# MiniMax-AI/VTP

Measured on NVIDIA H100. Metric: images/sec (256x256 encode+decode+3-loss step), higher is better.
Workload: dtype bf16

## Files before the change

vtp_b200/csrc/attention_bwd.cu:

```cuda
#include <stdlib.h>

#include "attention_bwd.cuh"
#include "host.h"
#include "ptx.cuh"

namespace vtp {

static constexpr int AB_THREADS = 384;
static constexpr int BQ = 0, BK_ = 32768, BV = 65536, BDO = 98304, BP = 131072, BDS = 163840, BX = 196608;
static constexpr int X_P0 = 0, X_DS0 = 1056, X_DK0 = 2112, X_DV0 = 2368, X_PCOL = 2624, X_DSCOL = 3648, X_BAR = 4672;
static constexpr int AB_SMEM = BX + X_BAR + 128 + 1024;

struct AttnBwdDev {
    const __nv_bfloat16* qkv;
    const __nv_bfloat16* o;
    const __nv_bfloat16* dout;
    const float* lse;
    __nv_bfloat16* dqkv;
    const __nv_bfloat16* rope_sin;
    const __nv_bfloat16* rope_cos;
    int B, T, H, D, prefix, HW, causal, nkt;
    float scale, scale_log2;
    int pack, rprefix;
};
// ... 271 lines not shown
                    if (kj < HW) {
                        float f[64];
                        load_row64(smem + BK_, kj, f);
                        float s = 0.f;
#pragma unroll
                        for (int d = 0; d < 64; ++d) s += q0[d] * f[d];
                        load_row64(smem + BV, kj, f);
                        float dp = 0.f;
#pragma unroll
                        for (int d = 0; d < 64; ++d) dp += do0[d] * f[d];
                        pv = ex2f(s * p.scale_log2 - lse0);
                        dsv = p.scale * pv * (dp - delta0);
                    }
                    p0[kj] = pv, ds0[kj] = dsv;
                }
            }
            __syncwarp();
            if (lane == 0) mbar_arrive(bar_cls);
            float kc[64], vc[64];
            load_grow64(p.qkv + row0 * 3 * D + D + h * 64, kc);
            load_grow64(p.qkv + row0 * 3 * D + 2 * D + h * 64, vc);
            float s00 = 0.f, dp00 = 0.f;
#pragma unroll
            for (int d = 0; d < 64; ++d) s00 += q0[d] * kc[d], dp00 += do0[d] * vc[d];
            const float p00 = ex2f(s00 * p.scale_log2 - lse0);
            const float ds00 = p.scale * p00 * (dp00 - delta0);
            float a0 = 0.f, a1 = 0.f;
            for (int kj = 0; kj < HW; ++kj) {
                const float dsv = ds0[kj];
                const uint32_t w = *reinterpret_cast<const uint32_t*>(smem + BK_ + sw_off(kj, 2 * lane));
                a0 += dsv * bf16_lo(w), a1 += dsv * bf16_hi(w);
            }
            {
                const uint32_t w = __ldg(reinterpret_cast<const uint32_t*>(p.qkv + row0 * 3 * D + D + h * 64) + lane);
                a0 += ds00 * bf16_lo(w), a1 += ds00 * bf16_hi(w);
            }
            *reinterpret_cast<uint32_t*>(p.dqkv + row0 * 3 * D + h * 64 + 2 * lane) = pack_bf16x2(a0, a1);
            if (lane == 0) p0[260] = p00, ds0[260] = ds00;
        }
    }

    __syncthreads();
    if (warp == 8 && prefix > 0) {
        const float p00 = p0[260], ds00 = ds0[260];
        const uint32_t wdo = __ldg(reinterpret_cast<const uint32_t*>(p.dout + row0 * D + h * 64) + lane);
        const uint32_t wq = __ldg(reinterpret_cast<const uint32_t*>(p.qkv + row0 * 3 * D + h * 64) + lane);
        const float v0 = dv0[2 * lane] + p00 * bf16_lo(wdo), v1 = dv0[2 * lane + 1] + p00 * bf16_hi(wdo);
        const float k0 = dk0[2 * lane] + ds00 * bf16_lo(wq), k1 = dk0[2 * lane + 1] + ds00 * bf16_hi(wq);
        *reinterpret_cast<uint32_t*>(p.dqkv + row0 * 3 * D + 2 * D + h * 64 + 2 * lane) = pack_bf16x2(v0, v1);
        *reinterpret_cast<uint32_t*>(p.dqkv + row0 * 3 * D + D + h * 64 + 2 * lane) = pack_bf16x2(k0, k1);
    }
}


}

using namespace vtp;

extern "C" int vtp_attention_bwd(const void* qkv, const void* o, const void* dout, const float* lse, void* dqkv,
                                 const void* rope_sin, const void* rope_cos, int B, int T, int H, int prefix, int causal,
                                 vtp_stream_t st) {
    VTP_CHECK_ARG(qkv && o && dout && lse && dqkv && B > 0 && T > 0 && H > 0, "attention_bwd: bad args");
    VTP_CHECK_ARG(prefix == 0 || prefix == 1, "attention_bwd: prefix must be 0 or 1");
    VTP_CHECK_ARG(!(prefix && causal), "attention_bwd: causal + prefix is not supported");
    VTP_CHECK_ARG((rope_sin == nullptr) == (rope_cos == nullptr), "attention_bwd: rope tables");
    const int HW = T - prefix;
    VTP_CHECK_ARG(HW >= 1 && HW <= 256, "attention_bwd: %d non-prefix tokens not in [1,256]", HW);
    VTP_CHECK_ARG(B <= 65535, "attention_bwd: grid too large");
    const int D = H * 64;
    AttnBwdDev p;
    p.qkv = (const __nv_bfloat16*)qkv, p.o = (const __nv_bfloat16*)o, p.dout = (const __nv_bfloat16*)dout;
    p.lse = lse, p.dqkv = (__nv_bfloat16*)dqkv;
    p.rope_sin = (const __nv_bfloat16*)rope_sin, p.rope_cos = (const __nv_bfloat16*)rope_cos;
    p.B = B, p.T = T, p.H = H, p.D = D, p.prefix = prefix, p.HW = HW, p.causal = causal;
    p.nkt = HW > 128 ? 2 : 1;
    p.scale = 0.125f, p.scale_log2 = 0.125f * 1.4426950408889634f;
    p.pack = 0, p.rprefix = prefix;
    if (!causal && T <= 64 && B > 1 && getenv("VTP_ATTN_NO_PACK") == nullptr) {
        p.pack = 128 / T;
        p.prefix = 0, p.HW = T, p.nkt = 1;
    }
    CUtensorMap tq, td;
    {
        uint64_t dims[2] = {(uint64_t)3 * D, (uint64_t)B * T}, strides[1] = {(uint64_t)3 * D * 2};
        uint32_t box[2] = {64, 128};
        int rc = make_tmap_bf16(&tq, qkv, 2, dims, strides, box);
        if (rc) return rc;
    }
    {
        uint64_t dims[2] = {(uint64_t)D, (uint64_t)B * T}, strides[1] = {(uint64_t)D * 2};
        uint32_t box[2] = {64, 128};
        int rc = make_tmap_bf16(&td, dout, 2, dims, strides, box);
        if (rc) return rc;
    }
    static bool configured = false;
    if (!configured) {
        VTP_CUDA(cudaFuncSetAttribute(attn_bwd_kernel<1>, cudaFuncAttributeMaxDynamicSharedMemorySize, AB_SMEM));
        VTP_CUDA(cudaFuncSetAttribute(attn_bwd_kernel<2>, cudaFuncAttributeMaxDynamicSharedMemorySize, AB_SMEM));
        configured = true;
    }
    const dim3 grid(H, p.pack ? ceil_div(B, p.pack) : B);
    if (p.nkt == 2) attn_bwd_kernel<2><<<grid, AB_THREADS, AB_SMEM, (cudaStream_t)st>>>(tq, td, p);
    else attn_bwd_kernel<1><<<grid, AB_THREADS, AB_SMEM, (cudaStream_t)st>>>(tq, td, p);
    VTP_LAUNCH_CHECK();
    return VTP_OK;
}
```

vtp_b200/csrc/attention_bwd.cuh:

```cuda
#pragma once
#include "ptx.cuh"

namespace vtp {

__device__ __forceinline__ float ex2f(float x) {
    float y;
    asm("ex2.approx.ftz.f32 %0, %1;" : "=f"(y) : "f"(x));
    return y;
}
__device__ __forceinline__ uint32_t sw_off(int row, int col) {
    return row * 128 + ((((col >> 3) ^ (row & 7)) << 4) | ((col & 7) << 1));
}
__device__ __forceinline__ void load_row64(const uint8_t* tile, int row, float (&f)[64]) {
#pragma unroll
    for (int c = 0; c < 8; ++c) {
        const uint4 w = *reinterpret_cast<const uint4*>(tile + sw_off(row, c * 8));
        f[c * 8 + 0] = bf16_lo(w.x), f[c * 8 + 1] = bf16_hi(w.x), f[c * 8 + 2] = bf16_lo(w.y), f[c * 8 + 3] = bf16_hi(w.y);
        f[c * 8 + 4] = bf16_lo(w.z), f[c * 8 + 5] = bf16_hi(w.z), f[c * 8 + 6] = bf16_lo(w.w), f[c * 8 + 7] = bf16_hi(w.w);
    }
}
__device__ __forceinline__ void load_grow64(const __nv_bfloat16* g, float (&f)[64]) {
    const uint4* p = reinterpret_cast<const uint4*>(g);
#pragma unroll
    for (int c = 0; c < 8; ++c) {
        const uint4 w = __ldg(p + c);
        f[c * 8 + 0] = bf16_lo(w.x), f[c * 8 + 1] = bf16_hi(w.x), f[c * 8 + 2] = bf16_lo(w.y), f[c * 8 + 3] = bf16_hi(w.y);
        f[c * 8 + 4] = bf16_lo(w.z), f[c * 8 + 5] = bf16_hi(w.z), f[c * 8 + 6] = bf16_lo(w.w), f[c * 8 + 7] = bf16_hi(w.w);
    }
}

__device__ __forceinline__ float quad_dot(const uint8_t* tile, int row, const __nv_bfloat16* g, int c4) {
    float acc = 0.f;
#pragma unroll
    for (int c = 0; c < 2; ++c) {
        const uint4 a = *reinterpret_cast<const uint4*>(tile + sw_off(row, 16 * c4 + 8 * c));
        const uint4 w = __ldg(reinterpret_cast<const uint4*>(g + 16 * c4 + 8 * c));
        const uint32_t aw[4] = {a.x, a.y, a.z, a.w}, ww[4] = {w.x, w.y, w.z, w.w};
#pragma unroll
        for (int e = 0; e < 4; ++e) acc += bf16_lo(aw[e]) * bf16_lo(ww[e]) + bf16_hi(aw[e]) * bf16_hi(ww[e]);
    }
    acc += __shfl_xor_sync(0xffffffffu, acc, 1);
    acc += __shfl_xor_sync(0xffffffffu, acc, 2);
    return acc;
}

__device__ __forceinline__ void rope_bwd_frag(float (&g)[16], const __nv_bfloat16* sin_row, const __nv_bfloat16* cos_row, int c4) {
#pragma unroll
    for (int jn = 0; jn < 4; ++jn) {
        const int d = 8 * jn + 2 * c4;
        const uint32_t s_lo = __ldg(reinterpret_cast<const uint32_t*>(sin_row + d));
        const uint32_t s_hi = __ldg(reinterpret_cast<const uint32_t*>(sin_row + d + 32));
        const uint32_t c_lo = __ldg(reinterpret_cast<const uint32_t*>(cos_row + d));
        const uint32_t c_hi = __ldg(reinterpret_cast<const uint32_t*>(cos_row + d + 32));
        const float sl[2] = {bf16_lo(s_lo), bf16_hi(s_lo)}, sh[2] = {bf16_lo(s_hi), bf16_hi(s_hi)};
        const float cl[2] = {bf16_lo(c_lo), bf16_hi(c_lo)}, ch[2] = {bf16_lo(c_hi), bf16_hi(c_hi)};
#pragma unroll
        for (int c = 0; c < 2; ++c) {
            const float a = g[2 * jn + c], b = g[2 * (jn + 4) + c];
            g[2 * jn + c] = a * cl[c] + b * sh[c];
            g[2 * (jn + 4) + c] = b * ch[c] - a * sl[c];
        }
    }
}

}
```

vtp_b200/csrc/attention_bwd_long.cu:

```cuda
#include "attention_bwd.cuh"
#include "host.h"
#include "ptx.cuh"

namespace vtp {

namespace {

constexpr int BL_THREADS = 384;
constexpr int BL_NSTAGE = 2;
constexpr int BL_TILE = 128 * 128;
constexpr int DQ_Q = 0, DQ_DO = BL_TILE, DQ_KV = 2 * BL_TILE, DQ_BAR = DQ_KV + BL_NSTAGE * 2 * BL_TILE;
constexpr int DQ_SMEM = DQ_BAR + 128 + 1024;
constexpr int KV_K = 0, KV_V = BL_TILE, KV_QD = 2 * BL_TILE, KV_LD = KV_QD + BL_NSTAGE * 2 * BL_TILE;
constexpr int KV_BAR = KV_LD + BL_NSTAGE * 1024;
constexpr int KV_SMEM = KV_BAR + 128 + 1024;
constexpr float LOG2E = 1.4426950408889634f;

struct AttnBwdLongDev {
    const __nv_bfloat16* qkv;
    const __nv_bfloat16* o;
    const __nv_bfloat16* dout;
    const float* lse;
    float* delta;
    __nv_bfloat16* dqkv;
    const __nv_bfloat16* rope_sin;
    const __nv_bfloat16* rope_cos;
    int B, T, H, D, prefix, HW;
    float scale, scale_log2;
};

__global__ void __launch_bounds__(256) attn_bwd_delta_kernel(const AttnBwdLongDev p) {
    const long gid = (long)blockIdx.x * blockDim.x + threadIdx.x;
    const long pair = gid >> 3;
    const int c = (int)(gid & 7);
    const bool valid = pair < (long)p.B * p.T * p.H;
    float acc = 0.f;
    if (valid) {
        const long tok = pair / p.H;
        const int h = (int)(pair - tok * p.H);
        const uint4 a = __ldg(reinterpret_cast<const uint4*>(p.dout + tok * p.D + h * 64) + c);
        const uint4 w = __ldg(reinterpret_cast<const uint4*>(p.o + tok * p.D + h * 64) + c);
        const uint32_t aw[4] = {a.x, a.y, a.z, a.w}, ww[4] = {w.x, w.y, w.z, w.w};
#pragma unroll
        for (int e = 0; e < 4; ++e) acc += bf16_lo(aw[e]) * bf16_lo(ww[e]) + bf16_hi(aw[e]) * bf16_hi(ww[e]);
    }
    acc += __shfl_xor_sync(0xffffffffu, acc, 1);
    acc += __shfl_xor_sync(0xffffffffu, acc, 2);
    acc += __shfl_xor_sync(0xffffffffu, acc, 4);
    if (valid && c == 0) {
        const long tok = pair / p.H;
        const int h = (int)(pair - tok * p.H);
        const long b = tok / p.T;
        p.delta[(b * p.H + h) * p.T + (tok - b * p.T)] = acc;
    }
}

__device__ __forceinline__ void pack_a(const float (&x)[32], uint32_t (&a)[4][4]) {
#pragma unroll
    for (int kk = 0; kk < 4; ++kk) {
        a[kk][0] = pack_bf16x2(x[8 * kk], x[8 * kk + 1]), a[kk][1] = pack_bf16x2(x[8 * kk + 2], x[8 * kk + 3]);
        a[kk][2] = pack_bf16x2(x[8 * kk + 4], x[8 * kk + 5]), a[kk][3] = pack_bf16x2(x[8 * kk + 6], x[8 * kk + 7]);
    }
}

__global__ void __launch_bounds__(BL_THREADS, 1) attn_bwd_long_dq_kernel(const __grid_constant__ CUtensorMap tm_qkv,
                                                                          const __grid_constant__ CUtensorMap tm_do,
                                                                          const AttnBwdLongDev p) {
    extern __shared__ uint8_t smem_raw[];
    uint8_t* smem = reinterpret_cast<uint8_t*>((reinterpret_cast<uintptr_t>(smem_raw) + 1023) & ~uintptr_t(1023));
    uint64_t* bars = reinterpret_cast<uint64_t*>(smem + DQ_BAR);
    uint64_t* bar_q = bars;
    uint64_t* full = bars + 1;
    uint64_t* empty = full + BL_NSTAGE;

    const int warp = threadIdx.x >> 5, lane = threadIdx.x & 31;
    const int qt = blockIdx.x, h = blockIdx.y, b = blockIdx.z;
    const int D = p.D, T = p.T, prefix = p.prefix, HW = p.HW;
    const long row0 = (long)b * T;
    const int nkt = (HW + 127) / 128;

    if (threadIdx.x == 0) {
        tma_prefetch_desc(&tm_qkv);
        tma_prefetch_desc(&tm_do);
        mbar_init(bar_q, 1);
        for (int s = 0; s < BL_NSTAGE; ++s) mbar_init(full + s, 1), mbar_init(empty + s, 8);
        fence_barrier_init();
    }
    __syncthreads();

    if (warp < 8) {
        setmaxnreg_inc<200>();
        const int wg = warp >> 2, tw = threadIdx.x & 127, c4 = lane & 3;
        int rr[2], qi[2];
        bool qvalid[2];
#pragma unroll
        for (int i = 0; i < 2; ++i) {
            rr[i] = 64 * wg + 16 * (tw >> 5) + (lane >> 2) + 8 * i;
            qi[i] = 128 * qt + rr[i];
            qvalid[i] = qi[i] < HW;
        }
        const __nv_bfloat16* kcls = p.qkv + row0 * 3 * D + D + h * 64;
        const __nv_bfloat16* vcls = p.qkv + row0 * 3 * D + 2 * D + h * 64;
        mbar_wait(bar_q, 0);
        float lsc[2], dl[2], ds_cls[2];
#pragma unroll
        for (int i = 0; i < 2; ++i) {
            const long li = ((long)b * p.H + h) * T + prefix + qi[i];
            lsc[i] = qvalid[i] ? p.lse[li] * LOG2E : 0.f;
            dl[i] = qvalid[i] ? p.delta[li] : 0.f;
            ds_cls[i] = 0.f;
            if (prefix > 0) {
                const float s0 = quad_dot(smem + DQ_Q, rr[i], kcls, c4);
                const float dp0 = quad_dot(smem + DQ_DO, rr[i], vcls, c4);
                if (qvalid[i]) ds_cls[i] = p.scale * ex2f(s0 * p.scale_log2 - lsc[i]) * (dp0 - dl[i]);
            }
        }
        float dq[32];
// ... 1 lines not shown
        for (int k = 0; k < 32; ++k) dq[k] = 0.f;
        const uint32_t aQ = smem_u32(smem + DQ_Q) + wg * 8192, aDO = smem_u32(smem + DQ_DO) + wg * 8192;
        for (int t = 0; t < nkt; ++t) {
            const int st = t % BL_NSTAGE;
            mbar_wait(full + st, (t / BL_NSTAGE) & 1);
            const uint32_t aK = smem_u32(smem + DQ_KV + st * 2 * BL_TILE), aV = aK + BL_TILE;
            const int klim = HW - 128 * t;
#pragma unroll 1
            for (int half = 0; half < 2 && 64 * half < klim; ++half) {
                float s[32], dp[32];
                wgmma_fence();
#pragma unroll
                for (int j = 0; j < 4; ++j)
                    wgmma_m64n64_ss<0, 0>(s, wgmma_desc_sw128(aQ + j * 32, 0, 1024),
                                          wgmma_desc_sw128(aK + half * 8192 + j * 32, 0, 1024), j > 0);
#pragma unroll
                for (int j = 0; j < 4; ++j)
                    wgmma_m64n64_ss<0, 0>(dp, wgmma_desc_sw128(aDO + j * 32, 0, 1024),
                                          wgmma_desc_sw128(aV + half * 8192 + j * 32, 0, 1024), j > 0);
                wgmma_commit();
                wgmma_wait<0>();
                fence_regs(s);
                fence_regs(dp);
#pragma unroll
                for (int jn = 0; jn < 8; ++jn)
#pragma unroll
                    for (int i = 0; i < 2; ++i)
#pragma unroll
                        for (int c = 0; c < 2; ++c) {
                            const int e = 4 * jn + 2 * i + c;
                            float de = 0.f;
                            if (qvalid[i] && 64 * half + 8 * jn + 2 * c4 + c < klim) {
                                const float pe = ex2f(s[e] * p.scale_log2 - lsc[i]);
                                de = p.scale * pe * (dp[e] - dl[i]);
                            }
                            s[e] = de;
                        }
                uint32_t a[4][4];
                pack_a(s, a);
                wgmma_fence();
#pragma unroll
                for (int kk = 0; kk < 4; ++kk)
                    wgmma_m64n64_rs<1>(dq, a[kk], wgmma_desc_sw128(aK + (4 * half + kk) * 2048, 8192, 1024), 1);
                wgmma_commit();
                wgmma_wait<0>();
                fence_regs(dq);
            }
            __syncwarp();
            if (lane == 0) mbar_arrive(empty + st);
        }
#pragma unroll
        for (int i = 0; i < 2; ++i) {
            if (!qvalid[i]) continue;
            float gq[16];
#pragma unroll
            for (int e = 0; e < 16; ++e) gq[e] = dq[4 * (e >> 1) + 2 * i + (e & 1)];
            if (prefix > 0) {
#pragma unroll
                for (int jn = 0; jn < 8; ++jn) {
                    const uint32_t w = __ldg(reinterpret_cast<const uint32_t*>(kcls + 8 * jn + 2 * c4));
                    gq[2 * jn] += ds_cls[i] * bf16_lo(w), gq[2 * jn + 1] += ds_cls[i] * bf16_hi(w);
                }
            }
            if (p.rope_sin) rope_bwd_frag(gq, p.rope_sin + (long)qi[i] * 64, p.rope_cos + (long)qi[i] * 64, c4);
            __nv_bfloat16* drow = p.dqkv + (row0 + prefix + qi[i]) * 3 * D + h * 64;
#pragma unroll
            for (int jn = 0; jn < 8; ++jn)
                *reinterpret_cast<uint32_t*>(drow + 8 * jn + 2 * c4) = pack_bf16x2(gq[2 * jn], gq[2 * jn + 1]);
        }
    } else {
        setmaxnreg_dec<104>();
        if (warp != 8 || lane != 0) return;
        const int row_k = (int)row0 + prefix;
        mbar_expect_tx(bar_q, 2 * BL_TILE);
        tma_load_2d(smem + DQ_Q, &tm_qkv, bar_q, h * 64, row_k + 128 * qt);
        tma_load_2d(smem + DQ_DO, &tm_do, bar_q, h * 64, row_k + 128 * qt);
        for (int t = 0; t < nkt; ++t) {
            const int st = t % BL_NSTAGE;
            if (t >= BL_NSTAGE) mbar_wait(empty + st, ((t / BL_NSTAGE) - 1) & 1);
            uint8_t* kv = smem + DQ_KV + st * 2 * BL_TILE;
            mbar_expect_tx(full + st, 2 * BL_TILE);
            tma_load_2d(kv, &tm_qkv, full + st, D + h * 64, row_k + 128 * t);
            tma_load_2d(kv + BL_TILE, &tm_qkv, full + st, 2 * D + h * 64, row_k + 128 * t);
        }
    }
}

__global__ void __launch_bounds__(BL_THREADS, 1) attn_bwd_long_dkdv_kernel(const __grid_constant__ CUtensorMap tm_qkv,
                                                                            const __grid_constant__ CUtensorMap tm_do,
                                                                            const AttnBwdLongDev p) {
    extern __shared__ uint8_t smem_raw[];
    uint8_t* smem = reinterpret_cast<uint8_t*>((reinterpret_cast<uintptr_t>(smem_raw) + 1023) & ~uintptr_t(1023));
    uint64_t* bars = reinterpret_cast<uint64_t*>(smem + KV_BAR);
    uint64_t* bar_kv = bars;
    uint64_t* full = bars + 1;
    uint64_t* empty = full + BL_NSTAGE;

    const int warp = threadIdx.x >> 5, lane = threadIdx.x & 31;
    const int kt = blockIdx.x, h = blockIdx.y, b = blockIdx.z;
    const int D = p.D, T = p.T, prefix = p.prefix, HW = p.HW;
    const long row0 = (long)b * T;
    const int nqt = (HW + 127) / 128;
    const long lrow = ((long)b * p.H + h) * T;

    if (threadIdx.x == 0) {
        tma_prefetch_desc(&tm_qkv);
        tma_prefetch_desc(&tm_do);
        mbar_init(bar_kv, 1);
        for (int s = 0; s < BL_NSTAGE; ++s) mbar_init(full + s, 1 + 32), mbar_init(empty + s, 8);
        fence_barrier_init();
    }
    __syncthreads();

    if (warp < 8) {
        setmaxnreg_inc<200>();
        const int wg = warp >> 2, tw = threadIdx.x & 127, c4 = lane & 3;
        int rr[2], kj[2];
        bool kvalid[2];
#pragma unroll
        for (int i = 0; i < 2; ++i) {
            rr[i] = 64 * wg + 16 * (tw >> 5) + (lane >> 2) + 8 * i;
// ... 30 lines not shown
#pragma unroll 1
            for (int half = 0; half < 2 && 64 * half < qlim; ++half) {
                float s[32], dp[32];
                wgmma_fence();
#pragma unroll
                for (int j = 0; j < 4; ++j)
                    wgmma_m64n64_ss<0, 0>(s, wgmma_desc_sw128(aK + j * 32, 0, 1024),
                                          wgmma_desc_sw128(aQ + half * 8192 + j * 32, 0, 1024), j > 0);
#pragma unroll
                for (int j = 0; j < 4; ++j)
                    wgmma_m64n64_ss<0, 0>(dp, wgmma_desc_sw128(aV + j * 32, 0, 1024),
                                          wgmma_desc_sw128(aDO + half * 8192 + j * 32, 0, 1024), j > 0);
                wgmma_commit();
                wgmma_wait<0>();
                fence_regs(s);
                fence_regs(dp);
#pragma unroll
                for (int jn = 0; jn < 8; ++jn)
#pragma unroll
                    for (int c = 0; c < 2; ++c) {
                        const int qc = 64 * half + 8 * jn + 2 * c4 + c;
                        const float lq = lse_s[qc], dq = dl_s[qc];
#pragma unroll
                        for (int i = 0; i < 2; ++i) {
                            const int e = 4 * jn + 2 * i + c;
                            float pe = 0.f, de = 0.f;
                            if (kvalid[i] && qc < qlim) {
                                pe = ex2f(s[e] * p.scale_log2 - lq);
                                de = p.scale * pe * (dp[e] - dq);
                            }
                            s[e] = pe, dp[e] = de;
                        }
                    }
                uint32_t ap[4][4], as[4][4];
                pack_a(s, ap);
                pack_a(dp, as);
                wgmma_fence();
#pragma unroll
                for (int kk = 0; kk < 4; ++kk) {
                    wgmma_m64n64_rs<1>(dv, ap[kk], wgmma_desc_sw128(aDO + (4 * half + kk) * 2048, 8192, 1024), 1);
                    wgmma_m64n64_rs<1>(dk, as[kk], wgmma_desc_sw128(aQ + (4 * half + kk) * 2048, 8192, 1024), 1);
                }
                wgmma_commit();
                wgmma_wait<0>();
                fence_regs(dv);
                fence_regs(dk);
            }
            __syncwarp();
            if (lane == 0) mbar_arrive(empty + st);
        }
#pragma unroll
        for (int i = 0; i < 2; ++i) {
            if (!kvalid[i]) continue;
            float gv[16], gk[16];
#pragma unroll
            for (int e = 0; e < 16; ++e) {
                const int jn = e >> 1, cc = e & 1;
                gv[e] = dv[4 * jn + 2 * i + cc], gk[e] = dk[4 * jn + 2 * i + cc];
            }
            if (prefix > 0) {
#pragma unroll
                for (int jn = 0; jn < 8; ++jn) {
                    const uint32_t wd = __ldg(reinterpret_cast<const uint32_t*>(docls + 8 * jn + 2 * c4));
                    const uint32_t wq = __ldg(reinterpret_cast<const uint32_t*>(qcls + 8 * jn + 2 * c4));
                    gv[2 * jn] += p0j[i] * bf16_lo(wd), gv[2 * jn + 1] += p0j[i] * bf16_hi(wd);
                    gk[2 * jn] += ds0j[i] * bf16_lo(wq), gk[2 * jn + 1] += ds0j[i] * bf16_hi(wq);
                }
            }
            if (p.rope_sin) rope_bwd_frag(gk, p.rope_sin + (long)kj[i] * 64, p.rope_cos + (long)kj[i] * 64, c4);
            __nv_bfloat16* drow = p.dqkv + (row0 + prefix + kj[i]) * 3 * D + h * 64;
#pragma unroll
            for (int jn = 0; jn < 8; ++jn) {
                *reinterpret_cast<uint32_t*>(drow + 2 * D + 8 * jn + 2 * c4) = pack_bf16x2(gv[2 * jn], gv[2 * jn + 1]);
                *reinterpret_cast<uint32_t*>(drow + D + 8 * jn + 2 * c4) = pack_bf16x2(gk[2 * jn], gk[2 * jn + 1]);
            }
        }
    } else {
        setmaxnreg_dec<104>();
        if (warp != 8) return;
        const int row_k = (int)row0 + prefix;
        if (lane == 0) {
            mbar_expect_tx(bar_kv, 2 * BL_TILE);
            tma_load_2d(smem + KV_K, &tm_qkv, bar_kv, D + h * 64, row_k + 128 * kt);
            tma_load_2d(smem + KV_V, &tm_qkv, bar_kv, 2 * D + h * 64, row_k + 128 * kt);
        }
        for (int t = 0; t < nqt; ++t) {
            const int st = t % BL_NSTAGE;
            if (t >= BL_NSTAGE) mbar_wait(empty + st, ((t / BL_NSTAGE) - 1) & 1);
            if (lane == 0) {
                uint8_t* qd = smem + KV_QD + st * 2 * BL_TILE;
                mbar_expect_tx(full + st, 2 * BL_TILE);
                tma_load_2d(qd, &tm_qkv, full + st, h * 64, row_k + 128 * t);
                tma_load_2d(qd + BL_TILE, &tm_do, full + st, h * 64, row_k + 128 * t);
            }
            float* lse_s = reinterpret_cast<float*>(smem + KV_LD + st * 1024);
#pragma unroll
            for (int r = lane; r < 128; r += 32) {
                const int q = 128 * t + r;
                lse_s[r] = q < HW ? p.lse[lrow + prefix + q] * LOG2E : 0.f;
                lse_s[128 + r] = q < HW ? p.delta[lrow + prefix + q] : 0.f;
            }
            mbar_arrive(full + st);
        }
    }
}

constexpr int PB_WARPS = 8;

__global__ void __launch_bounds__(PB_WARPS * 32) attn_bwd_prefix_kernel(const AttnBwdLongDev p) {
    __shared__ float cls[4][64];
    __shared__ float part[PB_WARPS][3][64];
    const int warp = threadIdx.x >> 5, lane = threadIdx.x & 31;
    const int h = blockIdx.x % p.H, b = blockIdx.x / p.H;
    const int D = p.D, T = p.T;
    const long row0 = (long)b * T, lrow = ((long)b * p.H + h) * T;
    const long rs = 3L * D;
    if (threadIdx.x < 256) {
        const int v = threadIdx.x >> 6, d = threadIdx.x & 63;
        const __nv_bfloat16* src = v < 3 ? p.qkv + row0 * rs + v * D + h * 64 : p.dout + row0 * D + h * 64;
        cls[v][d] = __bfloat162float(src[d]);
    }
    __syncthreads();
    const float lse0 = p.lse[lrow] * LOG2E, dl0 = p.delta[lrow];
    float aq0 = 0.f, aq1 = 0.f, ak0 = 0.f, ak1 = 0.f, av0 = 0.f, av1 = 0.f;
    for (int k0 = 32 * warp; k0 < T; k0 += 32 * PB_WARPS) {
        const int t = k0 + lane;
        float ds_0t = 0.f, ds_t0 = 0.f, p_t0 = 0.f;
        if (t < T) {
// ... 110 lines not shown
```

vtp_b200/csrc/ptx.cuh:

```cuda
#pragma once
#include <cuda_runtime.h>
#include <cuda_bf16.h>
#include <cuda.h>
#include <stdint.h>

namespace vtp {

__device__ __forceinline__ uint32_t smem_u32(const void* p) {
    return static_cast<uint32_t>(__cvta_generic_to_shared(p));
}
__device__ __forceinline__ uint32_t lane_id() { return threadIdx.x & 31; }

__device__ __forceinline__ bool elect_one() {
    uint32_t pred;
    asm volatile(
        "{\n\t.reg .pred p;\n\t"
        "elect.sync _|p, 0xffffffff;\n\t"
        "selp.u32 %0, 1, 0, p;\n\t}\n"
        : "=r"(pred));
    return pred != 0;
}

__device__ __forceinline__ void mbar_init(uint64_t* bar, uint32_t count) {
    asm volatile("mbarrier.init.shared::cta.b64 [%0], %1;" ::"r"(smem_u32(bar)), "r"(count));
}
__device__ __forceinline__ void fence_barrier_init() {
    asm volatile("fence.mbarrier_init.release.cluster;" ::: "memory");
}
__device__ __forceinline__ void mbar_expect_tx(uint64_t* bar, uint32_t bytes) {
    asm volatile("mbarrier.arrive.expect_tx.shared::cta.b64 _, [%0], %1;" ::"r"(smem_u32(bar)), "r"(bytes)
                 : "memory");
}
__device__ __forceinline__ void mbar_arrive(uint64_t* bar) {
    asm volatile("mbarrier.arrive.shared::cta.b64 _, [%0];" ::"r"(smem_u32(bar)) : "memory");
}
__device__ __forceinline__ bool mbar_try_wait(uint64_t* bar, uint32_t parity) {
    uint32_t ok;
    asm volatile(
        "{\n\t.reg .pred p;\n\t"
        "mbarrier.try_wait.parity.shared::cta.b64 p, [%1], %2;\n\t"
        "selp.u32 %0, 1, 0, p;\n\t}\n"
        : "=r"(ok)
        : "r"(smem_u32(bar)), "r"(parity)
        : "memory");
    return ok != 0;
}
__device__ __forceinline__ void mbar_wait(uint64_t* bar, uint32_t parity) {
    while (!mbar_try_wait(bar, parity)) {
    }
}

__device__ __forceinline__ void fence_proxy_async_smem() {
    asm volatile("fence.proxy.async.shared::cta;" ::: "memory");
}

__device__ __forceinline__ void tma_prefetch_desc(const CUtensorMap* m) {
    asm volatile("prefetch.tensormap [%0];" ::"l"(reinterpret_cast<uint64_t>(m)) : "memory");
}
__device__ __forceinline__ void tma_load_2d(void* dst, const CUtensorMap* m, uint64_t* bar, int x, int y) {
    asm volatile(
        "cp.async.bulk.tensor.2d.shared::cluster.global.mbarrier::complete_tx::bytes [%0], [%1, {%3, %4}], [%2];" ::
            "r"(smem_u32(dst)),
        "l"(reinterpret_cast<uint64_t>(m)), "r"(smem_u32(bar)), "r"(x), "r"(y)
        : "memory");
}
__device__ __forceinline__ void tma_load_3d(void* dst, const CUtensorMap* m, uint64_t* bar, int x, int y, int z) {
    asm volatile(
        "cp.async.bulk.tensor.3d.shared::cluster.global.mbarrier::complete_tx::bytes [%0], [%1, {%3, %4, %5}], [%2];" ::
            "r"(smem_u32(dst)),
        "l"(reinterpret_cast<uint64_t>(m)), "r"(smem_u32(bar)), "r"(x), "r"(y), "r"(z)
        : "memory");
}
__device__ __forceinline__ void tma_load_4d(void* dst, const CUtensorMap* m, uint64_t* bar, int x, int y, int z,
                                            int w) {
    asm volatile(
        "cp.async.bulk.tensor.4d.shared::cluster.global.mbarrier::complete_tx::bytes [%0], [%1, {%3, %4, %5, %6}], "
        "[%2];" ::"r"(smem_u32(dst)),
        "l"(reinterpret_cast<uint64_t>(m)), "r"(smem_u32(bar)), "r"(x), "r"(y), "r"(z), "r"(w)
        : "memory");
}

__device__ __forceinline__ void tma_store_2d(const CUtensorMap* m, const void* src, int x, int y) {
    asm volatile("cp.async.bulk.tensor.2d.global.shared::cta.bulk_group [%0, {%2, %3}], [%1];" ::"l"(
                     reinterpret_cast<uint64_t>(m)),
                 "r"(smem_u32(src)), "r"(x), "r"(y)
                 : "memory");
}
__device__ __forceinline__ void tma_store_4d(const CUtensorMap* m, const void* src, int x, int y, int z, int w) {
    asm volatile("cp.async.bulk.tensor.4d.global.shared::cta.bulk_group [%0, {%2, %3, %4, %5}], [%1];" ::"l"(
                     reinterpret_cast<uint64_t>(m)),
                 "r"(smem_u32(src)), "r"(x), "r"(y), "r"(z), "r"(w)
                 : "memory");
}
__device__ __forceinline__ void bulk_commit() { asm volatile("cp.async.bulk.commit_group;" ::: "memory"); }
__device__ __forceinline__ void bulk_wait_read0() { asm volatile("cp.async.bulk.wait_group.read 0;" ::: "memory"); }
__device__ __forceinline__ void bulk_wait0() { asm volatile("cp.async.bulk.wait_group 0;" ::: "memory"); }

__device__ __forceinline__ uint64_t wgmma_desc_sw128(uint32_t saddr, uint32_t lbo_bytes, uint32_t sbo_bytes) {
    uint64_t d = 0;
    d |= (uint64_t)((saddr & 0x3FFFF) >> 4);
    d |= (uint64_t)((lbo_bytes >> 4) & 0x3FFF) << 16;
    d |= (uint64_t)((sbo_bytes >> 4) & 0x3FFF) << 32;
// ... 79 lines not shown
```

Baseline: 600.9.

## Split non-causal attention backward over a 2-CTA cluster with DSMEM dQ reduction

Adds a new attention backward kernel for the HW>128 non-causal case. It launches 2-CTA clusters so each CTA owns 128 keys. dK/dV are computed per CTA with wgmma, and the partial dQ tiles are summed across the pair through distributed shared memory. Producer warps precompute lse, delta and the prefix (CLS) token terms, then reduce the CLS gradient across the cluster. This doubles the CTAs per head and batch to raise SM utilisation, at the cost of cluster syncs, DSMEM traffic and duplicated loads of Q and dO. Shared grad-row store and pack helpers are factored out.

```diff
diff --git a/vtp_b200/csrc/attention_bwd.cu b/vtp_b200/csrc/attention_bwd.cu
--- a/vtp_b200/csrc/attention_bwd.cu
+++ b/vtp_b200/csrc/attention_bwd.cu
@@ -347,6 +347,308 @@
     }
 }
 
+static constexpr int PR_K = 0, PR_V = 16384, PR_Q = 32768, PR_DO = 65536;
+static constexpr int PR_DS = 98304;
+static constexpr int PR_DQ = 131072;
+static constexpr int PR_SC = 196608;
+static constexpr int PR_RED = PR_SC + 4352;
+static constexpr int PR_BAR = PR_RED + 16 * 3 * 64 * 4;
+static constexpr int PR_SMEM = PR_BAR + 128 + 1024;
+
+__device__ __forceinline__ float dot8(uint4 a, uint4 b) {
+    return bf16_lo(a.x) * bf16_lo(b.x) + bf16_hi(a.x) * bf16_hi(b.x) + bf16_lo(a.y) * bf16_lo(b.y) +
+           bf16_hi(a.y) * bf16_hi(b.y) + bf16_lo(a.z) * bf16_lo(b.z) + bf16_hi(a.z) * bf16_hi(b.z) +
+           bf16_lo(a.w) * bf16_lo(b.w) + bf16_hi(a.w) * bf16_hi(b.w);
+}
+__device__ __forceinline__ float sum8(float x) {
+    x += __shfl_xor_sync(0xffffffffu, x, 1);
+    x += __shfl_xor_sync(0xffffffffu, x, 2);
+    return x + __shfl_xor_sync(0xffffffffu, x, 4);
+}
+__device__ __forceinline__ void axpy8(float (&acc)[8], float w, uint4 x) {
+    const uint32_t xs[4] = {x.x, x.y, x.z, x.w};
+#pragma unroll
+    for (int e = 0; e < 4; ++e) acc[2 * e] += w * bf16_lo(xs[e]), acc[2 * e + 1] += w * bf16_hi(xs[e]);
+}
+
+__global__ void __cluster_dims__(2, 1, 1) __launch_bounds__(AB_THREADS, 1)
+    attn_bwd_pair_kernel(const __grid_constant__ CUtensorMap tm_qkv, const __grid_constant__ CUtensorMap tm_do,
+                         const AttnBwdDev p) {
+    extern __shared__ uint8_t smem_raw[];
+    uint8_t* smem = reinterpret_cast<uint8_t*>((reinterpret_cast<uintptr_t>(smem_raw) + 1023) & ~uintptr_t(1023));
+    float* lse_s = reinterpret_cast<float*>(smem + PR_SC);
+    float* dl_s = lse_s + 256;
+    float* dsc_s = lse_s + 512;
+    float* psc_s = lse_s + 768;
+    float* cls_s = lse_s + 1024;
+    uint64_t* bars = reinterpret_cast<uint64_t*>(smem + PR_BAR);
+    uint64_t* bar_ld = bars;
+    uint64_t* bar_sc = bars + 2;
+
+    const int warp = threadIdx.x >> 5, lane = threadIdx.x & 31;
+    const int rank = (int)cluster_ctarank(), h = blockIdx.y, b = blockIdx.z;
+    const int D = p.D, T = p.T, prefix = p.prefix, HW = p.HW;
+    const long row0 = (long)b * T, lrow = ((long)b * p.H + h) * T;
+    const int nqt = (HW + 63) / 64;
+    const __nv_bfloat16* qcls = p.qkv + row0 * 3 * D + h * 64;
+    const __nv_bfloat16* kcls = qcls + D;
+    const __nv_bfloat16* vcls = qcls + 2 * D;
+    const __nv_bfloat16* docls = p.dout + row0 * D + h * 64;
+
+    if (threadIdx.x == 0) {
+        tma_prefetch_desc(&tm_qkv);
+        tma_prefetch_desc(&tm_do);
+        mbar_init(&bar_ld[0], 1), mbar_init(&bar_ld[1], 1);
+        for (int t = 0; t < 4; ++t) mbar_init(&bar_sc[t], 4);
+        fence_barrier_init();
+    }
+    __syncthreads();
+
+    if (warp < 8) {
+        setmaxnreg_inc<200>();
+        const int wg = __shfl_sync(0xffffffffu, warp >> 2, 0), tw = threadIdx.x & 127, c4 = lane & 3;
+        int rr[2], kj[2];
+        bool kvalid[2];
+#pragma unroll
+        for (int i = 0; i < 2; ++i) {
+            rr[i] = 64 * wg + 16 * (tw >> 5) + (lane >> 2) + 8 * i;
+            kj[i] = 128 * rank + rr[i];
+            kvalid[i] = kj[i] < HW;
+        }
+        mbar_wait(&bar_ld[0], 0);
+        mbar_wait(&bar_sc[0], 0);
+        float p0j[2] = {0.f, 0.f}, ds0j[2] = {0.f, 0.f};
+        if (prefix > 0) {
+#pragma unroll
+            for (int i = 0; i < 2; ++i) {
+                const float s = quad_dot(smem + PR_K, rr[i], qcls, c4);
+                const float dp = quad_dot(smem + PR_V, rr[i], docls, c4);
+                if (kvalid[i]) {
+                    p0j[i] = ex2f(s * p.scale_log2 - cls_s[0]);
+                    ds0j[i] = p.scale * p0j[i] * (dp - cls_s[1]);
+                }
+            }
+        }
+        float dk[32], dv[32];
+#pragma unroll
+        for (int k = 0; k < 32; ++k) dk[k] = 0.f, dv[k] = 0.f;
+        const uint32_t aK = smem_u32(smem + PR_K), aV = smem_u32(smem + PR_V);
+#pragma unroll 1
+        for (int t = 0; t < nqt; ++t) {
+            if (t == 2) mbar_wait(&bar_ld[1], 0);
+            mbar_wait(&bar_sc[t], 0);
+            const uint32_t aQ = smem_u32(smem + PR_Q) + t * 8192, aDO = smem_u32(smem + PR_DO) + t * 8192;
+            const uint32_t aDS = smem_u32(smem + PR_DS) + (t & 1) * 16384;
+            float s[32], dp[32];
+            wgmma_fence();
+#pragma unroll
+            for (int j = 0; j < 4; ++j)
+                wgmma_m64n64_ss<0, 0>(s, wgmma_desc_sw128(aK + wg * 8192 + j * 32, 0, 1024),
+                                      wgmma_desc_sw128(aQ + j * 32, 0, 1024), j > 0);
+#pragma unroll
+            for (int j = 0; j < 4; ++j)
+                wgmma_m64n64_ss<0, 0>(dp, wgmma_desc_sw128(aV + wg * 8192 + j * 32, 0, 1024),
+                                      wgmma_desc_sw128(aDO + j * 32, 0, 1024), j > 0);
+            wgmma_commit();
+            wgmma_wait<0>();
+            fence_regs(s);
+            fence_regs(dp);
+            const int qlim = HW - 64 * t;
+#pragma unroll
+            for (int jn = 0; jn < 8; ++jn)
+#pragma unroll
+                for (int c = 0; c < 2; ++c) {
+                    const int qc = 8 * jn + 2 * c4 + c;
+                    const float lq = lse_s[64 * t + qc], dq_ = dl_s[64 * t + qc];
+#pragma unroll
+                    for (int i = 0; i < 2; ++i) {
+                        const int e = 4 * jn + 2 * i + c;
+                        float pe = 0.f, de = 0.f;
+                        if (kvalid[i] && qc < qlim) {
+                            pe = ex2f(s[e] * p.scale_log2 - lq);
+                            de = p.scale * pe * (dp[e] - dq_);
+                        }
+                        s[e] = pe, dp[e] = de;
+                    }
+                }
+            uint32_t ap[4][4], as[4][4];
+            pack_a(s, ap);
+            pack_a(dp, as);
+            uint8_t* ds_blk = smem + PR_DS + (t & 1) * 16384 + wg * 8192;
+#pragma unroll
+            for (int kk = 0; kk < 4; ++kk)
+#pragma unroll
+                for (int q = 0; q < 4; ++q)
+                    *reinterpret_cast<uint32_t*>(ds_blk + sw_off(rr[q & 1] - 64 * wg, 16 * kk + 8 * (q >> 1) + 2 * c4)) =
+                        as[kk][q];
+            fence_proxy_async_smem();
+            wgmma_fence();
+#pragma unroll
+            for (int kk = 0; kk < 4; ++kk) {
+                wgmma_m64n64_rs<1>(dv, ap[kk], wgmma_desc_sw128(aDO + kk * 2048, 8192, 1024), 1);
+                wgmma_m64n64_rs<1>(dk, as[kk], wgmma_desc_sw128(aQ + kk * 2048, 8192, 1024), 1);
+            }
+            wgmma_commit();
+            asm volatile("bar.sync 1, 256;" ::: "memory");
+            if ((t & 1) == wg) {
+                float dq[32];
+#pragma unroll
+                for (int k = 0; k < 32; ++k) dq[k] = 0.f;
+#pragma unroll
+                for (int kk = 0; kk < 8; ++kk)
+                    wgmma_m64n64_ss<1, 1>(dq, wgmma_desc_sw128(aDS + kk * 2048, 8192, 1024),
+                                          wgmma_desc_sw128(aK + kk * 2048, 8192, 1024), kk > 0);
+                wgmma_commit();
+                wgmma_wait<0>();
+                fence_regs(dq);
+                float4* part = reinterpret_cast<float4*>(smem + PR_DQ + t * 16384);
+#pragma unroll
+                for (int k = 0; k < 8; ++k) part[k * 128 + tw] = make_float4(dq[4 * k], dq[4 * k + 1], dq[4 * k + 2], dq[4 * k + 3]);
+            } else {
+                wgmma_wait<0>();
+            }
+            fence_regs(dv);
+            fence_regs(dk);
+        }
+#pragma unroll
+        for (int i = 0; i < 2; ++i) {
+            if (!kvalid[i]) continue;
+            const bool rope = p.rope_sin != nullptr;
+            __nv_bfloat16* drow = p.dqkv + (row0 + prefix + kj[i]) * 3 * D + h * 64;
+            store_grad_row(dv, i, p0j[i], prefix > 0 ? docls : nullptr, nullptr, nullptr, drow + 2 * D, c4);
+            store_grad_row(dk, i, ds0j[i], prefix > 0 ? qcls : nullptr, rope ? p.rope_sin + (long)kj[i] * 64 : nullptr,
+                           rope ? p.rope_cos + (long)kj[i] * 64 : nullptr, drow + D, c4);
+        }
+        cluster_sync();
+        const int t = rank + 2 * wg;
+        if (t < nqt) {
+            float dq[32];
+            const uint32_t own = smem_u32(smem + PR_DQ + t * 16384) + tw * 16;
+            const uint32_t peer = mapa_shared(own, (uint32_t)rank ^ 1u);
+#pragma unroll
+            for (int k = 0; k < 8; ++k) {
+                const float4 a = *reinterpret_cast<const float4*>(smem + PR_DQ + t * 16384 + (k * 128 + tw) * 16);
+                const float4 r = ld_shared_cluster_f4(peer + k * 2048);
+                dq[4 * k] = a.x + r.x, dq[4 * k + 1] = a.y + r.y, dq[4 * k + 2] = a.z + r.z, dq[4 * k + 3] = a.w + r.w;
+            }
+#pragma unroll
+            for (int i = 0; i < 2; ++i) {
+                const int qi = 64 * t + 16 * (tw >> 5) + (lane >> 2) + 8 * i;
+                if (qi >= HW) continue;
+                const bool rope = p.rope_sin != nullptr;
+                store_grad_row(dq, i, dsc_s[qi], prefix > 0 ? kcls : nullptr, rope ? p.rope_sin + (long)qi * 64 : nullptr,
+                               rope ? p.rope_cos + (long)qi * 64 : nullptr,
+                               p.dqkv + (row0 + prefix + qi) * 3 * D + h * 64, c4);
+            }
+        }
+    } else {
+        setmaxnreg_dec<104>();
+        if (warp == 8 && lane == 0) {
+            const int r = (int)row0 + prefix;
+            mbar_expect_tx(&bar_ld[0], 4 * 16384);
+            tma_load_2d(smem + PR_K, &tm_qkv, &bar_ld[0], D + h * 64, r + 128 * rank);
+            tma_load_2d(smem + PR_V, &tm_qkv, &bar_ld[0], 2 * D + h * 64, r + 128 * rank);
+            tma_load_2d(smem + PR_Q, &tm_qkv, &bar_ld[0], h * 64, r);
+            tma_load_2d(smem + PR_DO, &tm_do, &bar_ld[0], h * 64, r);
+            mbar_expect_tx(&bar_ld[1], 2 * 16384);
+            tma_load_2d(smem + PR_Q + 16384, &tm_qkv, &bar_ld[1], h * 64, r + 128);
+            tma_load_2d(smem + PR_DO + 16384, &tm_do, &bar_ld[1], h * 64, r + 128);
+        }
+        __syncwarp();
+        const int pt = threadIdx.x - 256, c = pt & 7, grp = pt >> 3;
+        uint4 q0c = make_uint4(0, 0, 0, 0), do0c = q0c, k0c = q0c, v0c = q0c;
+        float lse0 = 0.f, dl0 = 0.f;
+        if (prefix > 0) {
+            q0c = __ldg(reinterpret_cast<const uint4*>(qcls) + c), k0c = __ldg(reinterpret_cast<const uint4*>(kcls) + c);
+            v0c = __ldg(reinterpret_cast<const uint4*>(vcls) + c), do0c = __ldg(reinterpret_cast<const uint4*>(docls) + c);
+            dl0 = sum8(dot8(do0c, __ldg(reinterpret_cast<const uint4*>(p.o + row0 * D + h * 64) + c)));
+            lse0 = p.lse[lrow] * LOG2E;
+            if (pt == 0) cls_s[0] = lse0, cls_s[1] = dl0;
+        }
+        for (int t = 0; t < nqt; ++t) {
+#pragma unroll 4
+            for (int ps = 0; ps < 4; ++ps) {
+                const int q = 64 * t + 16 * ps + grp;
+                const bool valid = q < HW;
+                const long tok = row0 + prefix + (valid ? q : 0);
+                const uint4 wd = __ldg(reinterpret_cast<const uint4*>(p.dout + tok * D + h * 64) + c);
+                const uint4 wo = __ldg(reinterpret_cast<const uint4*>(p.o + tok * D + h * 64) + c);
+                const float dl = sum8(dot8(wd, wo));
+                const float lq = valid ? p.lse[lrow + prefix + q] * LOG2E : 0.f;
+                float p_q0 = 0.f, ds_q0 = 0.f;
+                if (prefix > 0) {
+                    const uint4 wq = __ldg(reinterpret_cast<const uint4*>(p.qkv + tok * 3 * D + h * 64) + c);
+                    const float s_q0 = sum8(dot8(wq, k0c)), dp_q0 = sum8(dot8(wd, v0c));
+                    p_q0 = valid ? ex2f(s_q0 * p.scale_log2 - lq) : 0.f;
+                    ds_q0 = valid ? p.scale * p_q0 * (dp_q0 - dl) : 0.f;
+                }
+                if (c == 0) lse_s[q] = lq, dl_s[q] = valid ? dl : 0.f, dsc_s[q] = ds_q0, psc_s[q] = p_q0;
+            }
+            __syncwarp();
+            if (lane == 0) mbar_arrive(&bar_sc[t]);
+        }
+        float* red = reinterpret_cast<float*>(smem + PR_RED);
+        if (prefix > 0) {
+            float aq[8], ak[8], av[8];
+#pragma unroll
+            for (int e = 0; e < 8; ++e) aq[e] = 0.f, ak[e] = 0.f, av[e] = 0.f;
+            for (int t = rank; t < nqt; t += 2) {
+#pragma unroll 2
+                for (int ps = 0; ps < 4; ++ps) {
+                    const int q = 64 * t + 16 * ps + grp;
+                    const bool valid = q < HW;
+                    const long tok = row0 + prefix + (valid ? q : 0);
+                    const uint4* row = reinterpret_cast<const uint4*>(p.qkv + tok * 3 * D + h * 64);
+                    const uint4 wq = __ldg(row + c), wk = __ldg(row + D / 8 + c), wv = __ldg(row + D / 4 + c);
+                    const uint4 wd = __ldg(reinterpret_cast<const uint4*>(p.dout + tok * D + h * 64) + c);
+                    const float s_0q = sum8(dot8(q0c, wk)), dp_0q = sum8(dot8(do0c, wv));
+                    const float ds_0q = valid ? p.scale * ex2f(s_0q * p.scale_log2 - lse0) * (dp_0q - dl0) : 0.f;
+                    axpy8(aq, ds_0q, wk);
+                    axpy8(ak, dsc_s[q], wq);
+                    axpy8(av, psc_s[q], wd);
+                }
+            }
+#pragma unroll
+            for (int e = 0; e < 8; ++e)
+                red[grp * 192 + 8 * c + e] = aq[e], red[grp * 192 + 64 + 8 * c + e] = ak[e],
+                                  red[grp * 192 + 128 + 8 * c + e] = av[e];
+            asm volatile("bar.sync 2, 128;" ::: "memory");
+            float x[3] = {0.f, 0.f, 0.f};
+            if (pt < 64) {
+                for (int g = 0; g < 16; ++g)
+#pragma unroll
+                    for (int v = 0; v < 3; ++v) x[v] += red[g * 192 + 64 * v + pt];
+            }
+            asm volatile("bar.sync 2, 128;" ::: "memory");
+            if (pt < 64) red[pt] = x[0], red[64 + pt] = x[1], red[128 + pt] = x[2];
+        }
+        cluster_sync();
+        if (prefix > 0 && rank == 0 && pt < 64) {
+            const uint32_t peer = mapa_shared(smem_u32(red), 1u);
+            float x[3];
+#pragma unroll
+            for (int v = 0; v < 3; ++v) {
+                float r;
+                asm volatile("ld.shared::cluster.f32 %0, [%1];" : "=f"(r) : "r"(peer + (64 * v + pt) * 4) : "memory");
+                x[v] = red[64 * v + pt] + r;
+            }
+            float s00 = 0.f, dp00 = 0.f;
+#pragma unroll
+            for (int cc = 0; cc < 8; ++cc) {
+                s00 += dot8(__ldg(reinterpret_cast<const uint4*>(qcls) + cc), __ldg(reinterpret_cast<const uint4*>(kcls) + cc));
+                dp00 += dot8(__ldg(reinterpret_cast<const uint4*>(docls) + cc), __ldg(reinterpret_cast<const uint4*>(vcls) + cc));
+            }
+            const float p00 = ex2f(s00 * p.scale_log2 - lse0), ds00 = p.scale * p00 * (dp00 - dl0);
+            const int d = pt;
+            x[0] += ds00 * __bfloat162float(kcls[d]);
+            x[1] += ds00 * __bfloat162float(qcls[d]);
+            x[2] += p00 * __bfloat162float(docls[d]);
+            __nv_bfloat16* drow = p.dqkv + row0 * 3 * D + h * 64 + d;
+            drow[0] = __float2bfloat16_rn(x[0]), drow[D] = __float2bfloat16_rn(x[1]), drow[2 * D] = __float2bfloat16_rn(x[2]);
+        }
+    }
+    cluster_sync();
+}
 
 }
 
@@ -361,7 +663,7 @@
     VTP_CHECK_ARG((rope_sin == nullptr) == (rope_cos == nullptr), "attention_bwd: rope tables");
     const int HW = T - prefix;
     VTP_CHECK_ARG(HW >= 1 && HW <= 256, "attention_bwd: %d non-prefix tokens not in [1,256]", HW);
-    VTP_CHECK_ARG(B <= 65535, "attention_bwd: grid too large");
+    VTP_CHECK_ARG(B <= 65535 && H <= 65535, "attention_bwd: grid too large");
     const int D = H * 64;
     AttnBwdDev p;
     p.qkv = (const __nv_bfloat16*)qkv, p.o = (const __nv_bfloat16*)o, p.dout = (const __nv_bfloat16*)dout;
@@ -392,10 +694,12 @@
     if (!configured) {
         VTP_CUDA(cudaFuncSetAttribute(attn_bwd_kernel<1>, cudaFuncAttributeMaxDynamicSharedMemorySize, AB_SMEM));
         VTP_CUDA(cudaFuncSetAttribute(attn_bwd_kernel<2>, cudaFuncAttributeMaxDynamicSharedMemorySize, AB_SMEM));
+        VTP_CUDA(cudaFuncSetAttribute(attn_bwd_pair_kernel, cudaFuncAttributeMaxDynamicSharedMemorySize, PR_SMEM));
         configured = true;
     }
     const dim3 grid(H, p.pack ? ceil_div(B, p.pack) : B);
-    if (p.nkt == 2) attn_bwd_kernel<2><<<grid, AB_THREADS, AB_SMEM, (cudaStream_t)st>>>(tq, td, p);
+    if (p.nkt == 2 && !causal) attn_bwd_pair_kernel<<<dim3(2, H, B), AB_THREADS, PR_SMEM, (cudaStream_t)st>>>(tq, td, p);
+    else if (p.nkt == 2) attn_bwd_kernel<2><<<grid, AB_THREADS, AB_SMEM, (cudaStream_t)st>>>(tq, td, p);
     else attn_bwd_kernel<1><<<grid, AB_THREADS, AB_SMEM, (cudaStream_t)st>>>(tq, td, p);
     VTP_LAUNCH_CHECK();
     return VTP_OK;
diff --git a/vtp_b200/csrc/attention_bwd.cuh b/vtp_b200/csrc/attention_bwd.cuh
--- a/vtp_b200/csrc/attention_bwd.cuh
+++ b/vtp_b200/csrc/attention_bwd.cuh
@@ -2,6 +2,8 @@
 #include "ptx.cuh"
 
 namespace vtp {
+
+constexpr float LOG2E = 1.4426950408889634f;
 
 __device__ __forceinline__ float ex2f(float x) {
     float y;
@@ -63,4 +65,31 @@
     }
 }
 
+__device__ __forceinline__ void pack_a(const float (&x)[32], uint32_t (&a)[4][4]) {
+#pragma unroll
+    for (int kk = 0; kk < 4; ++kk) {
+        a[kk][0] = pack_bf16x2(x[8 * kk], x[8 * kk + 1]), a[kk][1] = pack_bf16x2(x[8 * kk + 2], x[8 * kk + 3]);
+        a[kk][2] = pack_bf16x2(x[8 * kk + 4], x[8 * kk + 5]), a[kk][3] = pack_bf16x2(x[8 * kk + 6], x[8 * kk + 7]);
+    }
 }
+
+__device__ __forceinline__ void store_grad_row(const float (&acc)[32], int i, float w, const __nv_bfloat16* cls,
+                                               const __nv_bfloat16* sin_row, const __nv_bfloat16* cos_row,
+                                               __nv_bfloat16* drow, int c4) {
+    float g[16];
+#pragma unroll
+    for (int e = 0; e < 16; ++e) g[e] = acc[4 * (e >> 1) + 2 * i + (e & 1)];
+    if (cls) {
+#pragma unroll
+        for (int jn = 0; jn < 8; ++jn) {
+            const uint32_t x = __ldg(reinterpret_cast<const uint32_t*>(cls + 8 * jn + 2 * c4));
+            g[2 * jn] += w * bf16_lo(x), g[2 * jn + 1] += w * bf16_hi(x);
+        }
+    }
+    if (sin_row) rope_bwd_frag(g, sin_row, cos_row, c4);
+#pragma unroll
+    for (int jn = 0; jn < 8; ++jn)
+        *reinterpret_cast<uint32_t*>(drow + 8 * jn + 2 * c4) = pack_bf16x2(g[2 * jn], g[2 * jn + 1]);
+}
+
+}
diff --git a/vtp_b200/csrc/attention_bwd_long.cu b/vtp_b200/csrc/attention_bwd_long.cu
--- a/vtp_b200/csrc/attention_bwd_long.cu
+++ b/vtp_b200/csrc/attention_bwd_long.cu
@@ -14,7 +14,6 @@
 constexpr int KV_K = 0, KV_V = BL_TILE, KV_QD = 2 * BL_TILE, KV_LD = KV_QD + BL_NSTAGE * 2 * BL_TILE;
 constexpr int KV_BAR = KV_LD + BL_NSTAGE * 1024;
 constexpr int KV_SMEM = KV_BAR + 128 + 1024;
-constexpr float LOG2E = 1.4426950408889634f;
 
 struct AttnBwdLongDev {
     const __nv_bfloat16* qkv;
@@ -55,14 +54,6 @@
     }
 }
 
-__device__ __forceinline__ void pack_a(const float (&x)[32], uint32_t (&a)[4][4]) {
-#pragma unroll
-    for (int kk = 0; kk < 4; ++kk) {
-        a[kk][0] = pack_bf16x2(x[8 * kk], x[8 * kk + 1]), a[kk][1] = pack_bf16x2(x[8 * kk + 2], x[8 * kk + 3]);
-        a[kk][2] = pack_bf16x2(x[8 * kk + 4], x[8 * kk + 5]), a[kk][3] = pack_bf16x2(x[8 * kk + 6], x[8 * kk + 7]);
-    }
-}
-
 __global__ void __launch_bounds__(BL_THREADS, 1) attn_bwd_long_dq_kernel(const __grid_constant__ CUtensorMap tm_qkv,
                                                                           const __grid_constant__ CUtensorMap tm_do,
                                                                           const AttnBwdLongDev p) {
@@ -170,21 +161,10 @@
 #pragma unroll
         for (int i = 0; i < 2; ++i) {
             if (!qvalid[i]) continue;
-            float gq[16];
-#pragma unroll
-            for (int e = 0; e < 16; ++e) gq[e] = dq[4 * (e >> 1) + 2 * i + (e & 1)];
-            if (prefix > 0) {
-#pragma unroll
-                for (int jn = 0; jn < 8; ++jn) {
-                    const uint32_t w = __ldg(reinterpret_cast<const uint32_t*>(kcls + 8 * jn + 2 * c4));
-                    gq[2 * jn] += ds_cls[i] * bf16_lo(w), gq[2 * jn + 1] += ds_cls[i] * bf16_hi(w);
-                }
-            }
-            if (p.rope_sin) rope_bwd_frag(gq, p.rope_sin + (long)qi[i] * 64, p.rope_cos + (long)qi[i] * 64, c4);
-            __nv_bfloat16* drow = p.dqkv + (row0 + prefix + qi[i]) * 3 * D + h * 64;
-#pragma unroll
-            for (int jn = 0; jn < 8; ++jn)
-                *reinterpret_cast<uint32_t*>(drow + 8 * jn + 2 * c4) = pack_bf16x2(gq[2 * jn], gq[2 * jn + 1]);
+            const bool rope = p.rope_sin != nullptr;
+            store_grad_row(dq, i, ds_cls[i], prefix > 0 ? kcls : nullptr, rope ? p.rope_sin + (long)qi[i] * 64 : nullptr,
+                           rope ? p.rope_cos + (long)qi[i] * 64 : nullptr,
+                           p.dqkv + (row0 + prefix + qi[i]) * 3 * D + h * 64, c4);
         }
     } else {
         setmaxnreg_dec<104>();
@@ -321,28 +301,11 @@
 #pragma unroll
         for (int i = 0; i < 2; ++i) {
             if (!kvalid[i]) continue;
-            float gv[16], gk[16];
-#pragma unroll
-            for (int e = 0; e < 16; ++e) {
-                const int jn = e >> 1, cc = e & 1;
-                gv[e] = dv[4 * jn + 2 * i + cc], gk[e] = dk[4 * jn + 2 * i + cc];
-            }
-            if (prefix > 0) {
-#pragma unroll
-                for (int jn = 0; jn < 8; ++jn) {
-                    const uint32_t wd = __ldg(reinterpret_cast<const uint32_t*>(docls + 8 * jn + 2 * c4));
-                    const uint32_t wq = __ldg(reinterpret_cast<const uint32_t*>(qcls + 8 * jn + 2 * c4));
-                    gv[2 * jn] += p0j[i] * bf16_lo(wd), gv[2 * jn + 1] += p0j[i] * bf16_hi(wd);
-                    gk[2 * jn] += ds0j[i] * bf16_lo(wq), gk[2 * jn + 1] += ds0j[i] * bf16_hi(wq);
-                }
-            }
-            if (p.rope_sin) rope_bwd_frag(gk, p.rope_sin + (long)kj[i] * 64, p.rope_cos + (long)kj[i] * 64, c4);
+            const bool rope = p.rope_sin != nullptr;
             __nv_bfloat16* drow = p.dqkv + (row0 + prefix + kj[i]) * 3 * D + h * 64;
-#pragma unroll
-            for (int jn = 0; jn < 8; ++jn) {
-                *reinterpret_cast<uint32_t*>(drow + 2 * D + 8 * jn + 2 * c4) = pack_bf16x2(gv[2 * jn], gv[2 * jn + 1]);
-                *reinterpret_cast<uint32_t*>(drow + D + 8 * jn + 2 * c4) = pack_bf16x2(gk[2 * jn], gk[2 * jn + 1]);
-            }
+            store_grad_row(dv, i, p0j[i], prefix > 0 ? docls : nullptr, nullptr, nullptr, drow + 2 * D, c4);
+            store_grad_row(dk, i, ds0j[i], prefix > 0 ? qcls : nullptr, rope ? p.rope_sin + (long)kj[i] * 64 : nullptr,
+                           rope ? p.rope_cos + (long)kj[i] * 64 : nullptr, drow + D, c4);
         }
     } else {
         setmaxnreg_dec<104>();
diff --git a/vtp_b200/csrc/ptx.cuh b/vtp_b200/csrc/ptx.cuh
--- a/vtp_b200/csrc/ptx.cuh
+++ b/vtp_b200/csrc/ptx.cuh
@@ -48,6 +48,28 @@
 __device__ __forceinline__ void mbar_wait(uint64_t* bar, uint32_t parity) {
     while (!mbar_try_wait(bar, parity)) {
     }
+}
+
+__device__ __forceinline__ uint32_t cluster_ctarank() {
+    uint32_t r;
+    asm volatile("mov.u32 %0, %%cluster_ctarank;" : "=r"(r));
+    return r;
+}
+__device__ __forceinline__ void cluster_sync() {
+    asm volatile("barrier.cluster.arrive.release.aligned;\n\tbarrier.cluster.wait.acquire.aligned;" ::: "memory");
+}
+__device__ __forceinline__ uint32_t mapa_shared(uint32_t saddr, uint32_t rank) {
+    uint32_t r;
+    asm volatile("mapa.shared::cluster.u32 %0, %1, %2;" : "=r"(r) : "r"(saddr), "r"(rank));
+    return r;
+}
+__device__ __forceinline__ float4 ld_shared_cluster_f4(uint32_t caddr) {
+    float4 v;
+    asm volatile("ld.shared::cluster.v4.f32 {%0, %1, %2, %3}, [%4];"
+                 : "=f"(v.x), "=f"(v.y), "=f"(v.z), "=f"(v.w)
+                 : "r"(caddr)
+                 : "memory");
+    return v;
 }
 
 __device__ __forceinline__ void fence_proxy_async_smem() {
```

Result: faster. 651.3 (median of 6 runs) (+8.4%).
